# deweylab/RSEM

Hardware: AMD Instinct MI355X
Metric: EM read-alignments/s (nnz x EM iterations per second), rsem-run-em theta-only rounds (higher is better)
Workload: dtype f64; 1 GPU; BASELINE configs[2] (PairedEndQModel-shaped, the north-star target config): EM matrix of 50000000 reads x 200000 transcripts, 570042118 alignments (11.40/read) per GPU, frozen conprb (rounds >= 12); synthetic_config=C3, kernel=0, parallelism=1 GPU

## Files before the change

### rsem_amd/csrc/em.hip

```cpp
#include <climits>
#include <cstdlib>
#include <cmath>
#include <type_traits>

#include "comm_internal.hpp"
#include "em_internal.hpp"
#include "upload.hpp"
#include "sell_layout.hpp"
#include "unit_groups.hpp"

namespace {

using rsem::kEpsilon;
using rsem::LanePlan;
using rsem::Loop;

constexpr int kMaxTimedRounds = 4096;
constexpr int kWindow = 2048;
static_assert(kWindow == kLayoutWindow, "the layout sorts reads apart and sizes windows for the E step's LDS window (sell_layout.hpp)");

constexpr int kTotSlots = 64;



// ... 216 lines not shown
    const int n = M + 1;
    const int per = (n + n_close - 1) / n_close;
    SliceWalk walk;
    walk.load(me * per, min(n, me * per + per), kBlock, cur, A.prev);
    const double extra_c = wave_sum(cur[n + lane]) + N0, sum_c = wave_sum(cur[n + kTotSlots + lane]) + N0;
    const double extra_p = wave_sum(A.prev[n + lane]) + N0, sum_p = wave_sum(A.prev[n + kTotSlots + lane]) + N0;
    CloseAcc acc;
    walk.each(cur, A.prev, [&](int i, double craw, double praw) {
        const double c = craw + (i == 0 ? extra_c : 0.0);
        A.prev[i] = 0.0;
        acc.add(c, c / sum_c, (praw + (i == 0 ? extra_p : 0.0)) / sum_p);
    });
    close_reduce(acc, scratch);
    if (threadIdx.x == 0 && close_arrive(A.ctrl, A.mirror, me, n_close, acc, A.stat_round, A.min_round, A.max_round))
        for (int k = 0; k < 2 * kTotSlots; k++) A.prev[n + k] = 0.0;
}

__global__ __launch_bounds__(kBlock) void k_solo_finish(int32_t M, double N0, const double* __restrict__ buf, double* theta, double* counts_last) {
    const int n = M + 1;
    const int lane = threadIdx.x & 63;
    const double extra0 = wave_sum(buf[n + lane]) + N0, sum = wave_sum(buf[n + kTotSlots + lane]) + N0;
    const int i = blockIdx.x * blockDim.x + threadIdx.x;
    if (i < n) {
        const double c = buf[i] + (i == 0 ? extra0 : 0.0);
        counts_last[i] = c;
        theta[i] = c / sum;
    }
}

#ifndef RSEM_FQ_DEPTH
#define RSEM_FQ_DEPTH 3
#endif
constexpr int kFarQDepth = RSEM_FQ_DEPTH;
template <bool kFC, bool kSolo = false, bool kFQ = false>
__global__ __launch_bounds__(kBlock) void k_estep_lane(
    const Shape* __restrict__ shapes, const Unit* __restrict__ units, uint32_t T, int M,
    const double* __restrict__ theta, const double* __restrict__ tsrc, double N0, const unsigned char* __restrict__ sval,
    const int16_t* __restrict__ sexp, const int32_t* __restrict__ ssid, const double* __restrict__ sncp,
    const unsigned long long* __restrict__ masks, double* counts, double* totals, const Ctrl* ctrl,
    unsigned long long* trace, SoloArgs solo = SoloArgs(), XArgs xa = XArgs(), StartList sl = StartList()) {
    if (ctrl->done) return;
    if (trace && threadIdx.x == 0) trace[2 * blockIdx.x] = wall_clock64();
    __shared__ double th_win[kWindow];
    __shared__ double cnt_win[kWindow];
    __shared__ int fq_sid[kFQ ? (kBlock / 64) * kFarQCap : 1];
    __shared__ double fq_val[kFQ ? (kBlock / 64) * kFarQCap : 1];
    __shared__ int fq_n[kBlock / 64];
    const Unit U = units[blockIdx.x];
    const int lane = threadIdx.x & 63;
    const int w = __builtin_amdgcn_readfirstlane((int)(threadIdx.x >> 6));
    FarQueue fq;
    if (kFQ) {
        fq.sid = fq_sid + w * kFarQCap;
        fq.val = fq_val + w * kFarQCap;
        fq.n = fq_n + w;
        if (lane == 0) fq_n[w] = 0;
    }
    __shared__ CloseScratch close_lds;
    if (kSolo && solo.stat_round > 0) solo_close_round(solo, M, N0, theta, &close_lds);
    double noise = 0.0, neff = 0.0;
    {
        const Shape& G = U.S;
        Shape S;
        S.plane_base = G.plane_base;
        S.slice_base = G.slice_base;
        S.n_slices = G.n_slices;
        S.row_base = 0;
        S.n_rows = 0;
        S.slot_base = G.slot_base;
        S.K = G.K;
        S.lg = G.lg;
        S.fmt = G.fmt;
        S.val_base = G.val_base;
        S.cut = G.cut;
        S.reserved = 0;
        const uint32_t u_end = S.slice_base + U.slice_begin + U.n_slices;
        const uint32_t s_begin = S.slice_base + U.slice_begin + (uint32_t)w * U.per_wave;
        const uint32_t s_end = min(u_end, s_begin + U.per_wave);
#define RSEM_ESTEP_BLOCK(KK, QQ, FF, XX) \
    estep_block<KK, kFC, QQ, (QQ ? kQ32Depth[KK - 1] : kF64Depth[KK - 1]), FF, XX>(S, s_begin, s_end, lane, U.base, U.span, theta, tsrc, N0, th_win, cnt_win, sval, sexp, ssid, sncp, masks, counts, noise, neff, M, xa, FarQueue(), sl)
#define RSEM_ESTEP_BLOCK_FQ(KK, QQ, XX) \
    estep_block<KK, kFC, QQ, kFarQDepth, true, XX, true>(S, s_begin, s_end, lane, U.base, U.span, theta, tsrc, N0, th_win, cnt_win, sval, sexp, ssid, sncp, masks, counts, noise, neff, M, xa, fq)
        const int code = (S.K - 1) | ((S.fmt == kFmtQ32 ? 1 : 0) << 2) | ((U.pad[0] != 0 ? 1 : 0) << 3) | (((!kFC && S.fmt == kFmtF64X) ? 1 : 0) << 4);
        if constexpr (kFQ) {
            if (s_begin < u_end) switch ((code & 7) | ((code >> 4) << 3)) {
                case 0: RSEM_ESTEP_BLOCK_FQ(1, false, false); break;
                case 1: RSEM_ESTEP_BLOCK_FQ(2, false, false); break;
                case 2: RSEM_ESTEP_BLOCK_FQ(3, false, false); break;
                case 3: RSEM_ESTEP_BLOCK_FQ(4, false, false); break;
                case 4: RSEM_ESTEP_BLOCK_FQ(1, true, false); break;
                case 5: RSEM_ESTEP_BLOCK_FQ(2, true, false); break;
                case 6: RSEM_ESTEP_BLOCK_FQ(3, true, false); break;
                case 7: RSEM_ESTEP_BLOCK_FQ(4, true, false); break;
                default:
                    if constexpr (!kFC) switch (code & 3) {
                        case 0: RSEM_ESTEP_BLOCK_FQ(1, false, true); break;
                        case 1: RSEM_ESTEP_BLOCK_FQ(2, false, true); break;
                        case 2: RSEM_ESTEP_BLOCK_FQ(3, false, true); break;
                        default: RSEM_ESTEP_BLOCK_FQ(4, false, true); break;
                    }
                    break;
            } else {
                const ThetaSrc th = theta_src<kFC>(theta, tsrc, N0, lane);
                stage_windows<kFC>(U.base, U.span, M, th, th_win, cnt_win);
            }
        } else
        if (s_begin < u_end) switch (code) {
            case 0: RSEM_ESTEP_BLOCK(1, false, false, false); break;
            case 1: RSEM_ESTEP_BLOCK(2, false, false, false); break;
            case 2: RSEM_ESTEP_BLOCK(3, false, false, false); break;
            case 3: RSEM_ESTEP_BLOCK(4, false, false, false); break;
            case 4: RSEM_ESTEP_BLOCK(1, true, false, false); break;
            case 5: RSEM_ESTEP_BLOCK(2, true, false, false); break;
            case 6: RSEM_ESTEP_BLOCK(3, true, false, false); break;
            case 7: RSEM_ESTEP_BLOCK(4, true, false, false); break;
            case 8: RSEM_ESTEP_BLOCK(1, false, true, false); break;
// ... 72 lines not shown
        if (kFused) spent[i] = 0.0;
        else counts[i] = 0.0;
        acc.add(c, th, old);
    });
    close_reduce(acc, &close_lds);
    if (threadIdx.x == 0 && close_arrive(ctrl, mirror, (int)blockIdx.x, nb, acc, round, min_round, max_round)) s_last = 1;
    __syncthreads();
    if (!kFused && s_last && threadIdx.x < 2 * kTotSlots) __hip_atomic_store(&totals[threadIdx.x], 0.0, __ATOMIC_RELAXED, __HIP_MEMORY_SCOPE_AGENT);
}

}


struct rsem_em_ctx {
    int device = 0;
    int32_t M = 0;
    uint64_t N1 = 0, nnz = 0;
    hipStream_t stream = nullptr;
    bool own_stream = true;
    uint64_t* d_row_ptr = nullptr;
    int32_t* d_sid = nullptr;
    double* d_cp = nullptr;
    double* d_ncp = nullptr;
    bool have_values = false;
    SellLayout L;
    unsigned char* d_sval = nullptr;
    double* d_sncp = nullptr;
    int16_t* d_sexp = nullptr;
    int* d_fill_err = nullptr;
    int value_bits = 64;
    int value_range_bits = 8;
    int short_last_plane = 1;
    int short_min_units = kShortClassMinUnits;
    int sid_start_list = 1;
    SidTraffic sid_traffic;
    bool layout_has_q32 = false;
    bool layout_ok = false;
    Unit* d_units = nullptr;
    std::vector<Unit> h_units;
    uint64_t long_nnz = 0;
    uint32_t* d_rank = nullptr;
    double *d_xextra = nullptr, *d_xinv = nullptr;
    int split_rows = 1;
    int split_policy = 1;
    uint32_t n_far_units = 0;
    unsigned long long n_stray_reads = 0;
    int tune_passes_left = 1;
    uint32_t n_units = 0;
    uint32_t n_units_main = 0;
    uint32_t n_units_compact = 0;
    uint32_t n_units_queued = 0;
    int far_queue = 1;
    hipStream_t stream_x = nullptr;
    hipEvent_t ev_x_fork = nullptr, ev_x_join = nullptr;
    int x_overlap = 0;
    double* d_theta[2] = {nullptr, nullptr};
    double* d_red3 = nullptr;
    double* d_red = nullptr;
    double* d_counts = nullptr;
    double* d_counts_last = nullptr;
    double* d_totals = nullptr;
    double* d_w = nullptr;
    double* d_wn = nullptr;
    Ctrl* d_ctrl = nullptr;
    int grid_long = 0;
    uint32_t forced_T = 0;
// ... 27 lines not shown
    c->n_units_compact = c->n_units_main;
    if (rsem::far_group_adopted(c->far_queue != 0, c->n_units_queued, c->n_units_main))
        c->n_units_compact = (uint32_t)(std::stable_partition(c->h_units.begin(), mid, [&](const Unit& u) { return !queued(u); }) - c->h_units.begin());
    if (c->n_units)
        RSEM_HIP_TRY(hipMemcpyAsync(c->d_units, c->h_units.data(), sizeof(Unit) * c->n_units, hipMemcpyHostToDevice, c->stream));
    RSEM_HIP_TRY(hipStreamSynchronize(c->stream));
    c->sid_traffic = SidTraffic();
    if (c->L.d_start_list) {
        const bool far = c->far_queue != 0 && c->n_units_compact < c->n_units_main;
        return sell_count_sid_traffic(c->L, c->d_units, c->n_units, far ? c->n_units_compact : 0u, far ? c->n_units_main : 0u, c->stream, c->sid_traffic);
    }
    return RSEM_OK;
}

bool start_list_on(const rsem_em_ctx* c) { return c->sid_start_list != 0 && c->L.d_start_list != nullptr; }
uint64_t sid_bytes_loaded(const rsem_em_ctx* c) {
    if (!start_list_on(c)) return c->L.n_sid_planes_loaded * 256;
    const SidTraffic& t = c->sid_traffic;
    return 256 * (t.first_planes + t.marked_planes) + 4 * (t.list_entries + t.list_slices);
}

struct LaneIO {
    const double* theta = nullptr;
    const double* tsrc = nullptr;
    double N0 = 0.0;
    double* counts = nullptr;
    double* totals = nullptr;
    unsigned long long* trace = nullptr;
    SoloArgs solo;
    XArgs xa;
};

using LaneKernel = decltype(&k_estep_lane<false, false, false>);
LaneKernel lane_kernel(Loop loop, bool far_queue) {
    if (loop == Loop::PLAIN) return far_queue ? k_estep_lane<false, false, true> : k_estep_lane<false, false, false>;
    if (far_queue) return k_estep_lane<true, false, true>;
    return loop == Loop::SOLO ? k_estep_lane<true, true, false> : k_estep_lane<true, false, false>;
}

void launch_lane(rsem_em_ctx* c, Loop loop, bool far_queue, uint32_t u0, uint32_t u1, hipStream_t s, const LaneIO& io) {
    if (u1 <= u0) return;
    const bool closes = loop == Loop::SOLO && !far_queue;
    StartList sl;
    if (!far_queue && start_list_on(c)) { sl.list = c->L.d_start_list; sl.off = c->L.d_start_off; }
    hipLaunchKernelGGL(lane_kernel(loop, far_queue), dim3(u1 - u0), dim3(kBlock), 0, s, c->L.d_shapes, c->d_units + u0, c->L.T, c->M, io.theta, io.tsrc,
                       io.N0, (const unsigned char*)c->d_sval, (const int16_t*)c->d_sexp, c->L.d_ssid, c->d_sncp, c->L.d_masks, io.counts,
                       io.totals, (const Ctrl*)c->d_ctrl, io.trace ? io.trace + 2 * (size_t)u0 : nullptr,
                       closes ? io.solo : SoloArgs(), io.xa, sl);
}

LanePlan plan_lanes(const rsem_em_ctx* c, Loop loop) {
    rsem::UnitGroups g;
    g.n = c->n_units; g.n_main = c->n_units_main; g.n_compact = c->n_units_compact;
    g.far_queue = c->far_queue != 0; g.x_overlap = c->x_overlap != 0; g.split_rows = c->L.n_x_rows != 0; g.stream_x = c->stream_x != nullptr;
    return rsem::plan_lane_launches(g, loop);
}
void launch_planned(rsem_em_ctx* c, const LanePlan& plan, Loop loop, hipStream_t st, const LaneIO& io) {
    for (int i = 0; i < plan.n; i++) launch_lane(c, loop, plan.at[i].far_queue, plan.at[i].u0, plan.at[i].u1, plan.at[i].second ? c->stream_x : st, io);
}
int fork_x(rsem_em_ctx* c, hipStream_t st) {
    RSEM_HIP_TRY(hipEventRecord(c->ev_x_fork, st));
    RSEM_HIP_TRY(hipStreamWaitEvent(c->stream_x, c->ev_x_fork, 0));
    return RSEM_OK;
}
int join_x(rsem_em_ctx* c, hipStream_t st) {
    RSEM_HIP_TRY(hipEventRecord(c->ev_x_join, c->stream_x));
    RSEM_HIP_TRY(hipStreamWaitEvent(st, c->ev_x_join, 0));
    return RSEM_OK;
}

int launch_estep(rsem_em_ctx* c, const double* d_theta, double* d_counts, hipStream_t st, double* d_totals, unsigned long long* d_trace = nullptr) {
    const Ctrl* ctrl = c->d_ctrl;
    const LanePlan plan = plan_lanes(c, Loop::PLAIN);
    hipStream_t sx = plan.x_second ? c->stream_x : st;
    LaneIO io;
    io.theta = d_theta; io.counts = d_counts; io.totals = d_totals; io.trace = d_trace;
    if (plan.fork_join) { int rc = fork_x(c, st); if (rc != RSEM_OK) return rc; }
    if (c->L.n_x_rows) {
// ... 259 lines not shown
    TRY_OR_FAIL(dmalloc(&c->d_cp, nnz));
    TRY_OR_FAIL(dmalloc(&c->d_ncp, N1));
    if ((rc = rsem::staged_h2d(c->d_row_ptr, row_ptr, sizeof(uint64_t) * (N1 + 1), c->stream)) != RSEM_OK) return fail(rc);
    if ((rc = rsem::staged_h2d(c->d_sid, sid, sizeof(int32_t) * nnz, c->stream)) != RSEM_OK) return fail(rc);
    if (conprb) {
        if ((rc = rsem::staged_h2d(c->d_cp, conprb, sizeof(double) * nnz, c->stream)) != RSEM_OK) return fail(rc);
        if ((rc = rsem::staged_h2d(c->d_ncp, ncp, sizeof(double) * N1, c->stream)) != RSEM_OK) return fail(rc);
        c->have_values = true;
    }
    for (int i = 0; i < 2; i++) TRY_OR_FAIL(dmalloc(&c->d_theta[i], (size_t)M + 1));
    TRY_OR_FAIL(dmalloc(&c->d_red3, 3 * ((size_t)M + 1 + 2 * kTotSlots)));
    c->d_red = c->d_red3;
    c->d_counts = c->d_red;
    c->d_totals = c->d_red + (size_t)M + 1;
    TRY_OR_FAIL(dmalloc(&c->d_counts_last, (size_t)M + 1));
    TRY_OR_FAIL(hipMemsetAsync(c->d_totals, 0, sizeof(double) * 2 * kTotSlots, c->stream));
    TRY_OR_FAIL(hipHostMalloc((void**)&c->mirror, sizeof(HostMirror), hipHostMallocDefault));
    memset(c->mirror, 0, sizeof(HostMirror));
    for (int i = 0; i < 2; i++) TRY_OR_FAIL(hipEventCreateWithFlags(&c->lag_ev[i], hipEventDisableTiming));
    {
        int least = 0, greatest = 0;
        TRY_OR_FAIL(hipDeviceGetStreamPriorityRange(&least, &greatest));
        TRY_OR_FAIL(hipStreamCreateWithPriority(&c->stream2, hipStreamNonBlocking, greatest));
    }
    for (int i = 0; i < 4; i++) {
        TRY_OR_FAIL(hipEventCreateWithFlags(&c->ev_e[i], hipEventDisableTiming));
        TRY_OR_FAIL(hipEventCreateWithFlags(&c->ev_s[i], hipEventDisableTiming));
    }
    TRY_OR_FAIL(dmalloc(&c->d_ctrl, 1));
    TRY_OR_FAIL(hipMemsetAsync(c->d_counts, 0, sizeof(double) * ((size_t)M + 1), c->stream));
    TRY_OR_FAIL(hipMemsetAsync(c->d_ctrl, 0, sizeof(Ctrl), c->stream));
    if (const char* e = getenv("RSEM_HIP_T")) c->forced_T = (uint32_t)atoi(e);
    if (const char* e = getenv("RSEM_HIP_SID_START_LIST")) c->sid_start_list = atoi(e) != 0;
    rc = build_layout(c);
    if (rc != RSEM_OK) return fail(rc);
    rsem::thread_stager().release();
#undef TRY_OR_FAIL
    *out = c;
    return RSEM_OK;
}

int rsem_em_set_values(rsem_em_ctx* c, const double* conprb, const double* ncp) {
    RSEM_REQUIRE(c && conprb && ncp, "NULL argument");
    RSEM_HIP_TRY(hipSetDevice(c->device));
    { int rc0 = ensure_csr(c); if (rc0 != RSEM_OK) return rc0; }
    if (c->nnz) RSEM_HIP_TRY(hipMemcpyAsync(c->d_cp, conprb, sizeof(double) * c->nnz, hipMemcpyHostToDevice, c->stream));
    if (c->N1) RSEM_HIP_TRY(hipMemcpyAsync(c->d_ncp, ncp, sizeof(double) * c->N1, hipMemcpyHostToDevice, c->stream));
    c->have_values = true;
    int rc = fill_values(c);
    if (rc != RSEM_OK) return rc;
    RSEM_HIP_TRY(hipStreamSynchronize(c->stream));
    return RSEM_OK;
}

int rsem_em_get_values(rsem_em_ctx* c, double* conprb, double* ncp) {
    RSEM_REQUIRE(c && conprb && ncp, "NULL argument");
    if (!c->have_values) { rsem::set_last_error("CSR values were never set"); return RSEM_ERR_STATE; }
    RSEM_HIP_TRY(hipSetDevice(c->device));
    { int rc0 = ensure_csr(c); if (rc0 != RSEM_OK) return rc0; }
    if (c->nnz) RSEM_HIP_TRY(hipMemcpyAsync(conprb, c->d_cp, sizeof(double) * c->nnz, hipMemcpyDeviceToHost, c->stream));
    if (c->N1) RSEM_HIP_TRY(hipMemcpyAsync(ncp, c->d_ncp, sizeof(double) * c->N1, hipMemcpyDeviceToHost, c->stream));
    RSEM_HIP_TRY(hipStreamSynchronize(c->stream));
    return RSEM_OK;
}

int rsem_em_shard_rows(uint64_t N1, const uint64_t* row_ptr, int world, uint64_t* bounds) {
// ... 56 lines not shown
        c->x_overlap = value == 2 ? 1 : 0;
        return rebuild_layout(c);
    }
    if (!strcmp(key, "split_rows")) {
        RSEM_REQUIRE(value == 0 || value == 1, "split_rows must be 0 or 1");
        if (c->split_rows == (int)value) return RSEM_OK;
        c->split_rows = (int)value;
        return rebuild_layout(c);
    }
    if (!strcmp(key, "value_bits") || !strcmp(key, "value_range_bits")) {
        const bool bits = !strcmp(key, "value_bits");
        if (bits) RSEM_REQUIRE(value == 64 || value == 32, "value_bits must be 64 or 32");
        else RSEM_REQUIRE(value >= 0 && value <= 24, "value_range_bits must be in 0..24");
        int& field = bits ? c->value_bits : c->value_range_bits;
        if (field == (int)value) return RSEM_OK;
        field = (int)value;
        if (c->value_bits == 64 && !c->layout_has_q32) return RSEM_OK;
        return rebuild_layout(c);
    }
    if (!strcmp(key, "short_last_plane") || !strcmp(key, "short_class_min_units")) {
        const bool sw = !strcmp(key, "short_last_plane");
        if (sw) RSEM_REQUIRE(value == 0 || value == 1, "short_last_plane must be 0 or 1");
        else RSEM_REQUIRE(value >= 1 && value <= 1000000, "short_class_min_units must be in 1..1000000");
        int& field = sw ? c->short_last_plane : c->short_min_units;
        if (field == (int)value) return RSEM_OK;
        field = (int)value;
        if (!sw && !c->short_last_plane) return RSEM_OK;
        { int rc0 = ensure_csr(c); if (rc0 != RSEM_OK) return rc0; }
        return rebuild_layout(c);
    }
    if (!strcmp(key, "sid_start_list")) {
        RSEM_REQUIRE(value == 0 || value == 1, "sid_start_list must be 0 or 1");
        c->sid_start_list = (int)value;
        return RSEM_OK;
    }
    if (!strcmp(key, "check_every")) {
        RSEM_REQUIRE(value >= 1 && value <= kHistCap / 4, "check_every out of range");
        c->check_every = (int)value;
        return RSEM_OK;
    }
    rsem::set_last_error("unknown option '%s'", key);
    return RSEM_ERR_INVALID;
}

int rsem_em_get_info(const rsem_em_ctx* c, const char* key, int64_t* value) {
    RSEM_REQUIRE(c && key && value, "NULL argument");
    if (!strcmp(key, "value_bits")) *value = c->value_bits;
    else if (!strcmp(key, "csr_released")) *value = c->csr_released ? 1 : 0;
    else if (!strcmp(key, "csr_bytes")) *value = (int64_t)(12 * c->nnz);
    else if (!strcmp(key, "value_range_bits")) *value = c->value_range_bits;
    else if (!strcmp(key, "far_units")) *value = c->n_far_units;
    else if (!strcmp(key, "units")) *value = c->n_units;
    else if (!strcmp(key, "units_compact")) *value = c->n_units_compact;
    else if (!strcmp(key, "units_main")) *value = c->n_units_main;
    else if (!strcmp(key, "units_queued")) *value = c->n_units_queued;
    else if (!strcmp(key, "unit_tables_agree")) {
        std::vector<Unit> d(c->n_units);
        if (c->n_units) {
            RSEM_HIP_TRY(hipSetDevice(c->device));
            RSEM_HIP_TRY(hipMemcpyAsync(d.data(), c->d_units, sizeof(Unit) * c->n_units, hipMemcpyDeviceToHost, c->stream));
            RSEM_HIP_TRY(hipStreamSynchronize(c->stream));
        }
        bool same = d.size() == c->h_units.size();
        for (size_t i = 0; same && i < d.size(); i++) same = same_unit(d[i], c->h_units[i]);
        *value = same ? 1 : 0;
    }
    else if (!strcmp(key, "stray_reads")) *value = (int64_t)c->n_stray_reads;
    else if (!strcmp(key, "reads_q32")) *value = c->L.n_q32_rows;
    else if (!strcmp(key, "reads_sliced")) *value = c->L.n_sell_rows;
    else if (!strcmp(key, "reads_long")) *value = c->L.n_long_rows;
    else if (!strcmp(key, "value_plane_bytes")) *value = (int64_t)c->L.val_bytes;
    else if (!strcmp(key, "value_plane_entries")) *value = (int64_t)c->L.n_val_entries;
    else if (!strcmp(key, "short_last_plane")) *value = c->short_last_plane;
    else if (!strcmp(key, "short_class_min_units")) *value = c->short_min_units;
    else if (!strcmp(key, "short_classes")) *value = (int64_t)__builtin_popcountll(c->L.short_classes);
    else if (!strcmp(key, "shapes")) *value = c->L.n_shapes;
    else if (!strcmp(key, "unit_bytes")) *value = (int64_t)sizeof(Unit);
    else if (!strcmp(key, "sid_plane_bytes")) *value = (int64_t)(c->L.n_planes * 256);
    else if (!strcmp(key, "slots")) *value = c->L.n_slots;
    else if (!strcmp(key, "sid_plane_bytes_loaded")) *value = (int64_t)sid_bytes_loaded(c);
    else if (!strcmp(key, "sid_start_list")) *value = c->sid_start_list;
    else if (!strcmp(key, "start_list_entries")) *value = (int64_t)c->L.n_start_entries;
    else if (!strcmp(key, "start_list_bytes")) *value = (int64_t)(c->L.d_start_list ? 4 * (c->L.n_start_entries + kStartListPad) + 4 * (uint64_t)c->L.n_slices : 0);
    else if (!strcmp(key, "sid_first_slice_planes")) *value = (int64_t)c->sid_traffic.first_planes;
    else if (!strcmp(key, "start_list_entries_loaded")) *value = (int64_t)c->sid_traffic.list_entries;
    else if (!strcmp(key, "start_list_slices")) *value = (int64_t)c->sid_traffic.list_slices;
    else if (!strcmp(key, "sid_marked_planes_far_queue")) *value = (int64_t)c->sid_traffic.marked_planes;
    else if (!strcmp(key, "slices")) *value = c->L.n_slices;
    else if (!strcmp(key, "split_rows")) *value = c->L.n_x_rows;
    else if (!strcmp(key, "far_entries")) *value = (int64_t)c->L.n_far;
    else if (!strcmp(key, "window_entries")) {
        int64_t w = 0;
        for (const Unit& u : c->h_units) w += u.span;
        *value = w;
    } else if (!strcmp(key, "physical_bytes_per_launch")) {
        int64_t w = 0;
        for (const Unit& u : c->h_units) w += u.span;
        const uint64_t long_nnz = c->long_nnz + (c->L.n_long_rows * 4ull) / 3;
        const uint64_t far_bytes = 28 * c->L.n_far + 40 * (uint64_t)c->L.n_x_slots;
        *value = (int64_t)(c->L.val_bytes + sid_bytes_loaded(c) + (uint64_t)c->L.n_slots * (8 + (c->layout_has_q32 ? 2 : 0)) +
                           (uint64_t)c->L.n_slices * 8 + (uint64_t)c->n_units * sizeof(Unit) + (uint64_t)w * 16 + 16 * ((uint64_t)c->M + 1)) +
                 (int64_t)(12 * long_nnz + far_bytes);
    }
    else { rsem::set_last_error("unknown info key '%s'", key); return RSEM_ERR_INVALID; }
    return RSEM_OK;
}

int rsem_em_debug_trace(rsem_em_ctx* c, const double* theta, unsigned long long* out, uint32_t* n_units_io) {
    RSEM_REQUIRE(c && theta && out && n_units_io, "NULL argument");
    RSEM_REQUIRE(c->have_values && c->layout_ok, "needs the LANE kernel with values set");
    RSEM_REQUIRE(*n_units_io >= c->n_units, "trace buffer too small");
    RSEM_HIP_TRY(hipSetDevice(c->device));
    unsigned long long* d = nullptr;
    RSEM_HIP_TRY(hipMalloc((void**)&d, sizeof(unsigned long long) * 2 * std::max<uint32_t>(c->n_units, 1)));
// ... 423 lines not shown
```

### rsem_amd/csrc/estep_block.hpp

```cpp
#pragma once
#include <type_traits>

#include "simt_macros.hpp"

RSEM_DEVFN double wave_sum(double v) {
#pragma unroll
    for (int d = 32; d >= 1; d >>= 1) v += RSEM_SHFL_XOR(v, d);
    return v;
}


struct ThetaSrc {
    const double* v;
    double extra0, sum;
};
template <bool kFC>
RSEM_DEVFN double theta_at(const ThetaSrc& t, int i) {
    if (!kFC) return t.v[i];
    return (t.v[i] + (i == 0 ? t.extra0 : 0.0)) / t.sum;
}
template <bool kFC>
RSEM_DEVFN ThetaSrc theta_src(const double* __restrict__ v, const double* __restrict__ tsrc, double N0, int lane);

template <bool kFC>
// ... 26 lines not shown
struct StartList {
    const int32_t* list = nullptr;
    const uint32_t* off = nullptr;
};

template <int K, bool kQ>
struct SliceRegs {
    int id[K];
    typename std::conditional<kQ, uint32_t, double>::type c[K];
    double nc;
    int e;
    double x;
    uint32_t slot0;
    double traw[K];
};

RSEM_DEVFN double pow2_of(int e) { return RSEM_LL_AS_DOUBLE((long long)(1023 + e) << 52); }

#ifndef RSEM_F64_DEPTHS
#define RSEM_F64_DEPTHS 2, 2, 2, 2
#endif
#ifndef RSEM_Q32_DEPTHS
#define RSEM_Q32_DEPTHS 2, 2, 2, 2
#endif
template <typename T>
RSEM_DEVFN T stream_load(const T* p) { return RSEM_NT_LOAD(p); }
template <int kCtrl>
RSEM_DEVFN double dpp_take(double v) {
    const long long b = RSEM_DOUBLE_AS_LL(v);
    const int lo = RSEM_DPP_MOV((int)(unsigned)b, kCtrl);
    const int hi = RSEM_DPP_MOV((int)(unsigned)(b >> 32), kCtrl);
    return RSEM_LL_AS_DOUBLE(((long long)hi << 32) | (unsigned)lo);
}
RSEM_DEVFN double read_sum_dpp(double part, int lg) {
    if (lg >= 1) part += dpp_take<0xB1>(part);
    if (lg >= 2) part += dpp_take<0x4E>(part);
    if (lg >= 3) part += dpp_take<0x141>(part);
    if (lg >= 4) part += dpp_take<0x140>(part);
    for (int d = 16; d < (1 << lg); d <<= 1) part += RSEM_SHFL_XOR(part, d);
    return part;
}
constexpr int kF64Depth[4] = {RSEM_F64_DEPTHS};
constexpr int kQ32Depth[4] = {RSEM_Q32_DEPTHS};

template <int K, bool kFC, bool kQ, int NBUF, bool kFar, bool kX = false, bool kFQ = false>
RSEM_DEVFN void estep_block(const Shape& S, uint32_t s_begin, uint32_t s_end, int lane, int base, int span,
                                   const double* __restrict__ theta, const double* __restrict__ tsrc, double N0, double* th_win, double* cnt_win,
                                   const unsigned char* __restrict__ sval, const int16_t* __restrict__ sexp, const int32_t* __restrict__ ssid,
                                   const double* __restrict__ sncp, const unsigned long long* __restrict__ masks,
                                   double* counts, double& noise, double& neff, int M, const XArgs& X = XArgs(), const FarQueue& FQ = FarQueue(),
                                   const StartList& SL = StartList()) {
    static_assert(!kFQ || kFar, "the far queue belongs to the loop of the units with ids outside their window");
    static_assert(!kFQ || NBUF >= 3, "the far-queue loop requests theta a slice ahead: three register sets at least (the ring loop)");
    using ValT = typename std::conditional<kQ, uint32_t, double>::type;
    const ValT* __restrict__ scp = (const ValT*)(sval + S.val_base);
    const int lg = S.lg;
    const int g = lane & ((1 << lg) - 1);
    const bool g0 = (g == 0);
    const uint32_t R = 64u >> lg;
    const bool kList = !kFQ && SL.list != nullptr;
    uint32_t m_base = s_begin;
    unsigned long long mv = (s_begin + lane < s_end) ? masks[s_begin + lane] : ~0ull;
    uint32_t ov = 0;
    if (kList) ov = (s_begin + lane < s_end) ? SL.off[s_begin + lane] : 0u;
    auto mask_of = [&](uint32_t t) -> unsigned long long {
        if (t - m_base >= 64u) {
            m_base = t;
            mv = (t + lane < s_end) ? masks[t + lane] : ~0ull;
            if (kList) { ov = (t + lane < s_end) ? SL.off[t + lane] : 0u; RSEM_PIN(ov); }
            RSEM_PIN(mv);
        }
        const int src = (int)(t - m_base);
        const uint32_t lo = RSEM_READLANE((int)(uint32_t)mv, src);
        const uint32_t hi = RSEM_READLANE((int)(uint32_t)(mv >> 32), src);
        return ((unsigned long long)hi << 32) | lo;
    };
    const unsigned ulane = (unsigned)lane, uslot = ulane >> lg;
    const unsigned Gk = (unsigned)shape_Gk(S);
    const unsigned last_lane = uslot * Gk + ((unsigned)g < Gk ? (unsigned)g : Gk - 1u);
    const bool last_ok = (unsigned)g < Gk;
    const uint32_t vstride = (uint32_t)RSEM_READFIRSTLANE((int)shape_val_stride(S));
    auto issue = [&](uint32_t t, unsigned long long m, SliceRegs<K, kQ>& b) {
        const uint32_t sl = t - S.slice_base;
        const uint64_t v0 = (uint64_t)sl * (K * 64);
        const ValT* __restrict__ vp = scp + (uint64_t)sl * vstride;
        if (kFQ || m != 0ull) {
            const int32_t* __restrict__ ip = ssid + (S.plane_base * 64 + v0);
            unsigned stride = 64u, idx = ulane;
            if (!kFQ) {
                const bool from_list = kList && t != s_begin;
                if (from_list) {
                    const uint32_t off = (uint32_t)RSEM_READLANE((int)ov, (int)(t - m_base));
                    const unsigned n = (unsigned)__builtin_popcountll(m);
                    const unsigned rank = (unsigned)RSEM_MBCNT((uint32_t)m, (uint32_t)(m >> 32));
                    ip = SL.list + off;
                    stride = n;
                    idx = rank < n ? rank : n - 1u;
                }
            }
#pragma unroll
            for (int k = 0; k < K; k++) b.id[k] = ip[(unsigned)k * stride + idx];
        }
#pragma unroll
        for (int k = 0; k < K - 1; k++) b.c[k] = stream_load(&vp[k * 64 + ulane]);
        b.c[K - 1] = stream_load(&vp[(K - 1) * 64 + last_lane]);
        const uint32_t slot0 = S.slot_base + sl * R;
        b.nc = (sncp + slot0)[uslot];
        b.e = kQ ? (int)(sexp + slot0)[uslot] : 0;
        b.x = kX ? (X.extra + (slot0 - X.slot_base))[uslot] : 0.0;
        b.slot0 = slot0;
    };
// ... 61 lines not shown
#pragma unroll
                    for (int k = 0; k < K; k++)
                        if (!((unsigned)(rsid[k] - base) < (unsigned)span))
                            rth[k] = kFC ? (cur.traw[k] + (rsid[k] == 0 ? th.extra0 : 0.0)) / th.sum : cur.traw[k];
                } else if (kFar && far) {
                    double t[K];
#pragma unroll
                    for (int k = 0; k < K; k++) {
                        const bool in = (unsigned)(rsid[k] - base) < (unsigned)span;
                        t[k] = theta_at<kFC>(th, in ? 0 : rsid[k]);
                    }
#pragma unroll
                    for (int k = 0; k < K; k++) {
                        RSEM_PIN(t[k]);
                        if (!((unsigned)(rsid[k] - base) < (unsigned)span)) rth[k] = t[k];
                    }
                }
            }
        }
        double f0 = g0 ? th0 * cur.nc : 0.0;
        if (f0 < kEpsilon) f0 = 0.0;
        double f[K];
        double part = f0 + ((kX && g0) ? cur.x : 0.0);
        const double scale = kQ ? pow2_of(cur.e) : 1.0;
#pragma unroll
        for (int k = 0; k < K; k++) {
            const ValT cr = (k == K - 1 && !last_ok) ? ValT(0) : cur.c[k];
            const double cv = kQ ? (double)cr * scale : (double)cr;
            double v = rth[k] * cv;
            if (v < kEpsilon) v = 0.0;
            f[k] = v;
            part += v;
        }
        part = read_sum_dpp(part, lg);
        const double inv = (part >= kEpsilon) ? 1.0 / part : 0.0;
        if (kX) RSEM_STORE_SAME(&(X.inv + (cur.slot0 - X.slot_base))[uslot], inv);
        noise += f0 * inv;
        neff += (g0 && part >= kEpsilon) ? 1.0 : 0.0;
#pragma unroll
        for (int k = 0; k < K; k++) acc[k] = acc[k] + f[k] * inv;
    };
    if constexpr (NBUF == 2) {
        SliceRegs<K, kQ> A, B;
        unsigned long long mA = ~0ull, mB = 0;
        issue(s_begin, mA, A);
        th = theta_src<kFC>(theta, tsrc, N0, lane);
        th0 = theta_at<kFC>(th, 0);
        stage_windows<kFC>(base, span, M, th, th_win, cnt_win);
        uint32_t s = s_begin;
        for (; s + 2 < s_end; s += 2) {
            mB = mask_of(s + 1);
            issue(s + 1, mB, B);
            reduce(A, mA);
            mA = mask_of(s + 2);
            issue(s + 2, mA, A);
            reduce(B, mB);
        }
        if (s + 1 < s_end) {
            mB = mask_of(s + 1);
            issue(s + 1, mB, B);
            reduce(A, mA);
            reduce(B, mB);
        } else {
            reduce(A, mA);
        }
    } else {
        SliceRegs<K, kQ> buf[NBUF];
        unsigned long long mk[NBUF];
// ... 51 lines not shown
```

### rsem_amd/csrc/sell_shape.hpp

```cpp
#pragma once

constexpr int kFmtF64 = 0, kFmtQ32 = 1, kFmtF64X = 2;
constexpr int kShapeTableMax = 148;

struct Shape {
    uint64_t plane_base;
    uint32_t slice_base;
    uint32_t n_slices;
    uint32_t row_base;
    uint32_t n_rows;
    uint32_t slot_base;
    int32_t K;
    int32_t lg;
    int32_t fmt;
    uint64_t val_base;
    int32_t cut;
    int32_t reserved;
};

__host__ __device__ inline uint32_t plane_bytes(int fmt) { return fmt == kFmtQ32 ? 256u : 512u; }

__host__ __device__ inline int shape_G(const Shape& S) {
    return 1 << S.lg;
}
__host__ __device__ inline uint32_t shape_R(const Shape& S) {
    return 64u >> S.lg;
}

__host__ __device__ inline uint32_t shape_val_stride(int K, int cut) {
    return (uint32_t)(K * 64 - 16 * cut);
}
__host__ __device__ inline uint32_t shape_val_stride(const Shape& S) { return shape_val_stride(S.K, S.cut); }
__host__ __device__ inline int shape_Gk(int lg, int cut) {
    return ((1 << lg) * (4 - cut)) >> 2;
}
__host__ __device__ inline int shape_Gk(const Shape& S) { return shape_Gk(S.lg, S.cut); }
__host__ __device__ inline uint32_t shape_val_off(int lg, int K, int cut, uint32_t r, int c, bool* ok = nullptr) {
    const int k = c >> lg, g = c & ((1 << lg) - 1);
    if (k < K - 1 || cut == 0) {
        if (ok) *ok = k < K;
        return (uint32_t)k * 64u + (r << lg) + (uint32_t)g;
    }
    const int Gk = shape_Gk(lg, cut);
    if (ok) *ok = k == K - 1 && g < Gk;
    return (uint32_t)(K - 1) * 64u + r * (uint32_t)Gk + (uint32_t)g;
}
__host__ __device__ inline uint32_t shape_val_off(const Shape& S, uint32_t r, int c, bool* ok = nullptr) {
    return shape_val_off(S.lg, S.K, S.cut, r, c, ok);
}
__host__ __device__ inline uint64_t shape_val_bytes(const Shape& S) {
    return (uint64_t)S.n_slices * shape_val_stride(S) * (plane_bytes(S.fmt) / 64u);
}

__host__ __device__ inline void row_to_slot(const Shape& S, uint32_t T, uint32_t q, uint32_t& slice_local, uint32_t& r) {
    const uint32_t R = shape_R(S), rpb = R * T;
    const uint32_t b = q / rpb, qb = q % rpb;
    const uint32_t left = S.n_rows - b * rpb;
    const uint32_t nb = left < rpb ? left : rpb;
    const uint32_t Tb = (nb + R - 1) / R;
// ... 5 lines not shown
```

### rsem_amd/csrc/simt_macros.hpp

```cpp
#pragma once
#ifndef RSEM_EMU
#define RSEM_DEVFN __device__ inline
#define RSEM_TIDX ((int)threadIdx.x)
#define RSEM_BDIM ((int)blockDim.x)
#define RSEM_SYNC() __syncthreads()
#define RSEM_SHFL_XOR(v, d) __shfl_xor(v, d)
#define RSEM_SHFL_DOWN(v, d) __shfl_down(v, d)
#define RSEM_SHFL_UP(v, d) __shfl_up(v, d)
#define RSEM_SHFL(v, src) __shfl(v, src)
#define RSEM_BALLOT(p) __ballot(p)
#define RSEM_READLANE(v, src) __builtin_amdgcn_readlane(v, src)
#define RSEM_ATOMIC_ADD(p, v) unsafeAtomicAdd(p, v)
#define RSEM_ATOMIC_ADD_I32(p, v) atomicAdd(p, v)
#define RSEM_LDS_ADD(p, v) (void)__builtin_amdgcn_ds_atomic_fadd_f64((__attribute__((address_space(3))) double*)(p), v)
#define RSEM_LDS_ADD_I32(p, v) (void)__hip_atomic_fetch_add((__attribute__((address_space(3))) int*)(p), v, __ATOMIC_RELAXED, __HIP_MEMORY_SCOPE_WORKGROUP)
#define RSEM_LDS_FETCH_ADD_I32(p, v) __hip_atomic_fetch_add((__attribute__((address_space(3))) int*)(p), v, __ATOMIC_RELAXED, __HIP_MEMORY_SCOPE_WORKGROUP)
#define RSEM_WAVE_SYNC()                                        \
    do {                                                        \
        __builtin_amdgcn_fence(__ATOMIC_RELEASE, "wavefront");  \
        __builtin_amdgcn_wave_barrier();                        \
        __builtin_amdgcn_fence(__ATOMIC_ACQUIRE, "wavefront");  \
    } while (0)
#define RSEM_WAIT_VM0() __builtin_amdgcn_s_waitcnt(0x0F70)
#define RSEM_READFIRSTLANE(v) __builtin_amdgcn_readfirstlane(v)
#define RSEM_MBCNT(lo, hi) __builtin_amdgcn_mbcnt_hi(hi, __builtin_amdgcn_mbcnt_lo(lo, 0u))
#define RSEM_PIN(x) asm volatile("" : "+v"(x))
#define RSEM_SCHED_FENCE() __builtin_amdgcn_sched_barrier(0)
#define RSEM_RCP(x) __builtin_amdgcn_rcp(x)
#define RSEM_DPP_MOV(v, ctrl) __builtin_amdgcn_update_dpp(0, v, ctrl, 0xf, 0xf, false)
#define RSEM_LL_AS_DOUBLE(x) __longlong_as_double(x)
#define RSEM_DOUBLE_AS_LL(x) __double_as_longlong(x)
#define RSEM_STORE_SAME(p, v) (*(p) = (v))
#define RSEM_NT_LOAD(p) __builtin_nontemporal_load(p)
#define RSEM_AGENT_LOAD(p) __hip_atomic_load(p, __ATOMIC_RELAXED, __HIP_MEMORY_SCOPE_AGENT)
#define RSEM_AGENT_STORE(p, v) __hip_atomic_store(p, v, __ATOMIC_RELAXED, __HIP_MEMORY_SCOPE_AGENT)
#define RSEM_AGENT_EXCHANGE(p, v) __hip_atomic_exchange(p, v, __ATOMIC_RELAXED, __HIP_MEMORY_SCOPE_AGENT)
#define RSEM_AGENT_FETCH_ADD(p, v) __hip_atomic_fetch_add(p, v, __ATOMIC_RELAXED, __HIP_MEMORY_SCOPE_AGENT)
#define RSEM_AGENT_FETCH_MAX(p, v) __hip_atomic_fetch_max(p, v, __ATOMIC_RELAXED, __HIP_MEMORY_SCOPE_AGENT)
#define RSEM_HOST_RELEASE_STORE(p, v) __hip_atomic_store(p, v, __ATOMIC_RELEASE, __HIP_MEMORY_SCOPE_SYSTEM)
#define RSEM_ZERO_DEP(z, x) asm volatile("v_and_b32 %0, 0, %1" : "=v"(z) : "v"(x))
#else
#ifndef RSEM_MBCNT
#define RSEM_MBCNT(lo, hi) __builtin_popcountll((((unsigned long long)(hi) << 32) | (unsigned long long)(lo)) & ((1ull << emu::lane()) - 1ull))
#endif
#endif
```

Baseline: 651.3 billion read-alignments/s.

## Specialise compact E-step kernels on compile-time lane-group width

```diff
diff --git a/rsem_amd/csrc/em.hip b/rsem_amd/csrc/em.hip
--- a/rsem_amd/csrc/em.hip
+++ b/rsem_amd/csrc/em.hip
@@ -272,7 +272,7 @@
 #define RSEM_FQ_DEPTH 3
 #endif
 constexpr int kFarQDepth = RSEM_FQ_DEPTH;
-template <bool kFC, bool kSolo = false, bool kFQ = false>
+template <bool kFC, bool kSolo = false, bool kFQ = false, bool kSpec = false>
 __global__ __launch_bounds__(kBlock) void k_estep_lane(
     const Shape* __restrict__ shapes, const Unit* __restrict__ units, uint32_t T, int M,
     const double* __restrict__ theta, const double* __restrict__ tsrc, double N0, const unsigned char* __restrict__ sval,
@@ -322,6 +322,32 @@
 #define RSEM_ESTEP_BLOCK_FQ(KK, QQ, XX) \
     estep_block<KK, kFC, QQ, kFarQDepth, true, XX, true>(S, s_begin, s_end, lane, U.base, U.span, theta, tsrc, N0, th_win, cnt_win, sval, sexp, ssid, sncp, masks, counts, noise, neff, M, xa, fq)
         const int code = (S.K - 1) | ((S.fmt == kFmtQ32 ? 1 : 0) << 2) | ((U.pad[0] != 0 ? 1 : 0) << 3) | (((!kFC && S.fmt == kFmtF64X) ? 1 : 0) << 4);
+        static_assert(!(kFQ && kSpec), "the far-queue loop reads the lane count from the shape");
+        bool spec_done = false;
+        if constexpr (kSpec) {
+            if (s_begin < u_end && code < 8 && lane_spec_pair(S.K, S.lg)) {
+                spec_done = true;
+#define RSEM_SPEC_CASE(KK, LL, QQ)                                                         \
+    case (QQ ? kShapesPerFmt : 0) + LL * 4 + KK - 1:                                       \
+        static_assert(lane_spec_pair(KK, LL), "an instantiation for a pair no layout holds"); \
+        estep_block<KK, kFC, QQ, (QQ ? kQ32Depth[KK - 1] : kF64Depth[KK - 1]), false, false, false, LL>(S, s_begin, s_end, lane, U.base, U.span, theta, tsrc, N0, th_win, cnt_win, sval, sexp, ssid, sncp, masks, counts, noise, neff, M, xa, FarQueue(), sl); \
+        break;
+#define RSEM_SPEC_CASES(QQ)                                                                                            \
+    RSEM_SPEC_CASE(1, 0, QQ) RSEM_SPEC_CASE(2, 0, QQ) RSEM_SPEC_CASE(3, 0, QQ) RSEM_SPEC_CASE(4, 0, QQ)                \
+    RSEM_SPEC_CASE(3, 1, QQ) RSEM_SPEC_CASE(4, 1, QQ) RSEM_SPEC_CASE(3, 2, QQ) RSEM_SPEC_CASE(4, 2, QQ)                \
+    RSEM_SPEC_CASE(3, 3, QQ) RSEM_SPEC_CASE(4, 3, QQ) RSEM_SPEC_CASE(3, 4, QQ) RSEM_SPEC_CASE(4, 4, QQ)                \
+    RSEM_SPEC_CASE(3, 5, QQ) RSEM_SPEC_CASE(4, 5, QQ) RSEM_SPEC_CASE(3, 6, QQ) RSEM_SPEC_CASE(4, 6, QQ)
+                switch ((S.fmt == kFmtQ32 ? kShapesPerFmt : 0) + S.lg * 4 + S.K - 1) {
+                    RSEM_SPEC_CASES(false)
+                    RSEM_SPEC_CASES(true)
+                    default: spec_done = false; break;
+                }
+#undef RSEM_SPEC_CASES
+#undef RSEM_SPEC_CASE
+            }
+        }
+        if (spec_done) {
+        } else
         if constexpr (kFQ) {
             if (s_begin < u_end) switch ((code & 7) | ((code >> 4) << 3)) {
                 case 0: RSEM_ESTEP_BLOCK_FQ(1, false, false); break;
@@ -460,6 +486,7 @@
     int value_range_bits = 8;
     int short_last_plane = 1;
     int short_min_units = kShortClassMinUnits;
+    int lane_spec = 1;
     int sid_start_list = 1;
     SidTraffic sid_traffic;
     bool layout_has_q32 = false;
@@ -553,10 +580,11 @@
 };
 
 using LaneKernel = decltype(&k_estep_lane<false, false, false>);
-LaneKernel lane_kernel(Loop loop, bool far_queue) {
-    if (loop == Loop::PLAIN) return far_queue ? k_estep_lane<false, false, true> : k_estep_lane<false, false, false>;
+LaneKernel lane_kernel(Loop loop, bool far_queue, bool spec) {
+    if (loop == Loop::PLAIN) return far_queue ? k_estep_lane<false, false, true> : (spec ? k_estep_lane<false, false, false, true> : k_estep_lane<false, false, false>);
     if (far_queue) return k_estep_lane<true, false, true>;
-    return loop == Loop::SOLO ? k_estep_lane<true, true, false> : k_estep_lane<true, false, false>;
+    if (loop == Loop::SOLO) return spec ? k_estep_lane<true, true, false, true> : k_estep_lane<true, true, false>;
+    return spec ? k_estep_lane<true, false, false, true> : k_estep_lane<true, false, false>;
 }
 
 void launch_lane(rsem_em_ctx* c, Loop loop, bool far_queue, uint32_t u0, uint32_t u1, hipStream_t s, const LaneIO& io) {
@@ -564,7 +592,7 @@
     const bool closes = loop == Loop::SOLO && !far_queue;
     StartList sl;
     if (!far_queue && start_list_on(c)) { sl.list = c->L.d_start_list; sl.off = c->L.d_start_off; }
-    hipLaunchKernelGGL(lane_kernel(loop, far_queue), dim3(u1 - u0), dim3(kBlock), 0, s, c->L.d_shapes, c->d_units + u0, c->L.T, c->M, io.theta, io.tsrc,
+    hipLaunchKernelGGL(lane_kernel(loop, far_queue, c->lane_spec != 0), dim3(u1 - u0), dim3(kBlock), 0, s, c->L.d_shapes, c->d_units + u0, c->L.T, c->M, io.theta, io.tsrc,
                        io.N0, (const unsigned char*)c->d_sval, (const int16_t*)c->d_sexp, c->L.d_ssid, c->d_sncp, c->L.d_masks, io.counts,
                        io.totals, (const Ctrl*)c->d_ctrl, io.trace ? io.trace + 2 * (size_t)u0 : nullptr,
                        closes ? io.solo : SoloArgs(), io.xa, sl);
@@ -890,6 +918,7 @@
     TRY_OR_FAIL(hipMemsetAsync(c->d_ctrl, 0, sizeof(Ctrl), c->stream));
     if (const char* e = getenv("RSEM_HIP_T")) c->forced_T = (uint32_t)atoi(e);
     if (const char* e = getenv("RSEM_HIP_SID_START_LIST")) c->sid_start_list = atoi(e) != 0;
+    if (const char* e = getenv("RSEM_HIP_LANE_SPEC")) c->lane_spec = atoi(e) != 0;
     rc = build_layout(c);
     if (rc != RSEM_OK) return fail(rc);
     rsem::thread_stager().release();
@@ -1012,6 +1041,11 @@
     if (!strcmp(key, "sid_start_list")) {
         RSEM_REQUIRE(value == 0 || value == 1, "sid_start_list must be 0 or 1");
         c->sid_start_list = (int)value;
+        return RSEM_OK;
+    }
+    if (!strcmp(key, "lane_spec")) {
+        RSEM_REQUIRE(value == 0 || value == 1, "lane_spec must be 0 or 1");
+        c->lane_spec = (int)value;
         return RSEM_OK;
     }
     if (!strcmp(key, "check_every")) {
@@ -1060,6 +1094,24 @@
     else if (!strcmp(key, "slots")) *value = c->L.n_slots;
     else if (!strcmp(key, "sid_plane_bytes_loaded")) *value = (int64_t)sid_bytes_loaded(c);
     else if (!strcmp(key, "sid_start_list")) *value = c->sid_start_list;
+    else if (!strcmp(key, "lane_spec")) *value = c->lane_spec;
+    else if (!strcmp(key, "lane_spec_pairs") || !strcmp(key, "lane_spec_pairs_in_units")) {
+        const bool in_units = key[15] != 0;
+        int64_t bits = 0;
+        if (!in_units) {
+            for (int lg = 0; lg <= 6; lg++)
+                for (int K = 1; K <= kMaxK; K++)
+                    if (lane_spec_pair(K, lg)) bits |= (1ll << (lg * 4 + K - 1)) | (1ll << (kShapesPerFmt + lg * 4 + K - 1));
+        } else {
+            const size_t n = std::min<size_t>(c->h_units.size(), c->n_units_compact);
+            for (size_t i = 0; i < n; i++) {
+                const Unit& U = c->h_units[i];
+                if (U.pad[0] == 0 && (U.S.fmt == kFmtF64 || U.S.fmt == kFmtQ32) && lane_spec_pair(U.S.K, U.S.lg))
+                    bits |= 1ll << ((U.S.fmt == kFmtQ32 ? kShapesPerFmt : 0) + U.S.lg * 4 + U.S.K - 1);
+            }
+        }
+        *value = bits;
+    }
     else if (!strcmp(key, "start_list_entries")) *value = (int64_t)c->L.n_start_entries;
     else if (!strcmp(key, "start_list_bytes")) *value = (int64_t)(c->L.d_start_list ? 4 * (c->L.n_start_entries + kStartListPad) + 4 * (uint64_t)c->L.n_slices : 0);
     else if (!strcmp(key, "sid_first_slice_planes")) *value = (int64_t)c->sid_traffic.first_planes;
diff --git a/rsem_amd/csrc/estep_block.hpp b/rsem_amd/csrc/estep_block.hpp
--- a/rsem_amd/csrc/estep_block.hpp
+++ b/rsem_amd/csrc/estep_block.hpp
@@ -82,7 +82,17 @@
     const int hi = RSEM_DPP_MOV((int)(unsigned)(b >> 32), kCtrl);
     return RSEM_LL_AS_DOUBLE(((long long)hi << 32) | (unsigned)lo);
 }
+template <int LG = -1>
 RSEM_DEVFN double read_sum_dpp(double part, int lg) {
+    if constexpr (LG >= 0) {
+        if constexpr (LG >= 1) part += dpp_take<0xB1>(part);
+        if constexpr (LG >= 2) part += dpp_take<0x4E>(part);
+        if constexpr (LG >= 3) part += dpp_take<0x141>(part);
+        if constexpr (LG >= 4) part += dpp_take<0x140>(part);
+        if constexpr (LG >= 5) part += RSEM_SHFL_XOR(part, 16);
+        if constexpr (LG >= 6) part += RSEM_SHFL_XOR(part, 32);
+        return part;
+    }
     if (lg >= 1) part += dpp_take<0xB1>(part);
     if (lg >= 2) part += dpp_take<0x4E>(part);
     if (lg >= 3) part += dpp_take<0x141>(part);
@@ -90,10 +100,19 @@
     for (int d = 16; d < (1 << lg); d <<= 1) part += RSEM_SHFL_XOR(part, d);
     return part;
 }
+RSEM_DEVFN double recip_of_normaliser(double x) {
+    double y = RSEM_RCP(x);
+    double e = RSEM_FMA(-x, y, 1.0);
+    y = RSEM_FMA(y, e, y);
+    e = RSEM_FMA(-x, y, 1.0);
+    y = RSEM_FMA(y, e, y);
+    const double r = RSEM_FMA(-x, y, 1.0);
+    return RSEM_FMA(r, y, y);
+}
 constexpr int kF64Depth[4] = {RSEM_F64_DEPTHS};
 constexpr int kQ32Depth[4] = {RSEM_Q32_DEPTHS};
 
-template <int K, bool kFC, bool kQ, int NBUF, bool kFar, bool kX = false, bool kFQ = false>
+template <int K, bool kFC, bool kQ, int NBUF, bool kFar, bool kX = false, bool kFQ = false, int LG = -1>
 RSEM_DEVFN void estep_block(const Shape& S, uint32_t s_begin, uint32_t s_end, int lane, int base, int span,
                                    const double* __restrict__ theta, const double* __restrict__ tsrc, double N0, double* th_win, double* cnt_win,
                                    const unsigned char* __restrict__ sval, const int16_t* __restrict__ sexp, const int32_t* __restrict__ ssid,
@@ -102,9 +121,10 @@
                                    const StartList& SL = StartList()) {
     static_assert(!kFQ || kFar, "the far queue belongs to the loop of the units with ids outside their window");
     static_assert(!kFQ || NBUF >= 3, "the far-queue loop requests theta a slice ahead: three register sets at least (the ring loop)");
+    static_assert(LG < 0 || (LG <= 6 && !kFar && !kX && !kFQ), "the lane count is compiled into the compact loops only");
     using ValT = typename std::conditional<kQ, uint32_t, double>::type;
     const ValT* __restrict__ scp = (const ValT*)(sval + S.val_base);
-    const int lg = S.lg;
+    const int lg = LG >= 0 ? LG : S.lg;
     const int g = lane & ((1 << lg) - 1);
     const bool g0 = (g == 0);
     const uint32_t R = 64u >> lg;
@@ -126,7 +146,7 @@
         return ((unsigned long long)hi << 32) | lo;
     };
     const unsigned ulane = (unsigned)lane, uslot = ulane >> lg;
-    const unsigned Gk = (unsigned)shape_Gk(S);
+    const unsigned Gk = (unsigned)shape_Gk(lg, S.cut);
     const unsigned last_lane = uslot * Gk + ((unsigned)g < Gk ? (unsigned)g : Gk - 1u);
     const bool last_ok = (unsigned)g < Gk;
     const uint32_t vstride = (uint32_t)RSEM_READFIRSTLANE((int)shape_val_stride(S));
@@ -254,8 +274,8 @@
             f[k] = v;
             part += v;
         }
-        part = read_sum_dpp(part, lg);
-        const double inv = (part >= kEpsilon) ? 1.0 / part : 0.0;
+        part = read_sum_dpp<LG>(part, lg);
+        const double inv = (part >= kEpsilon) ? (LG >= 0 ? recip_of_normaliser(part) : 1.0 / part) : 0.0;
         if (kX) RSEM_STORE_SAME(&(X.inv + (cur.slot0 - X.slot_base))[uslot], inv);
         noise += f0 * inv;
         neff += (g0 && part >= kEpsilon) ? 1.0 : 0.0;
diff --git a/rsem_amd/csrc/sell_shape.hpp b/rsem_amd/csrc/sell_shape.hpp
--- a/rsem_amd/csrc/sell_shape.hpp
+++ b/rsem_amd/csrc/sell_shape.hpp
@@ -25,6 +25,10 @@
 }
 __host__ __device__ inline uint32_t shape_R(const Shape& S) {
     return 64u >> S.lg;
+}
+
+__host__ __device__ constexpr bool lane_spec_pair(int K, int lg) {
+    return lg == 0 ? (K >= 1 && K <= 4) : (lg >= 1 && lg <= 6 && (K == 3 || K == 4));
 }
 
 __host__ __device__ inline uint32_t shape_val_stride(int K, int cut) {
diff --git a/rsem_amd/csrc/simt_macros.hpp b/rsem_amd/csrc/simt_macros.hpp
--- a/rsem_amd/csrc/simt_macros.hpp
+++ b/rsem_amd/csrc/simt_macros.hpp
@@ -27,7 +27,8 @@
 #define RSEM_PIN(x) asm volatile("" : "+v"(x))
 #define RSEM_SCHED_FENCE() __builtin_amdgcn_sched_barrier(0)
 #define RSEM_RCP(x) __builtin_amdgcn_rcp(x)
-#define RSEM_DPP_MOV(v, ctrl) __builtin_amdgcn_update_dpp(0, v, ctrl, 0xf, 0xf, false)
+#define RSEM_DPP_MOV(v, ctrl) __builtin_amdgcn_mov_dpp(v, ctrl, 0xf, 0xf, false)
+#define RSEM_FMA(a, b, c) __builtin_fma(a, b, c)
 #define RSEM_LL_AS_DOUBLE(x) __longlong_as_double(x)
 #define RSEM_DOUBLE_AS_LL(x) __double_as_longlong(x)
 #define RSEM_STORE_SAME(p, v) (*(p) = (v))
@@ -40,6 +41,9 @@
 #define RSEM_HOST_RELEASE_STORE(p, v) __hip_atomic_store(p, v, __ATOMIC_RELEASE, __HIP_MEMORY_SCOPE_SYSTEM)
 #define RSEM_ZERO_DEP(z, x) asm volatile("v_and_b32 %0, 0, %1" : "=v"(z) : "v"(x))
 #else
+#ifndef RSEM_FMA
+#define RSEM_FMA(a, b, c) __builtin_fma(a, b, c)
+#endif
 #ifndef RSEM_MBCNT
 #define RSEM_MBCNT(lo, hi) __builtin_popcountll((((unsigned long long)(hi) << 32) | (unsigned long long)(lo)) & ((1ull << emu::lane()) - 1ull))
 #endif
```

Result: no change. 649.1 billion read-alignments/s, median of 2 (-0.3%).
